# farhiongit/aho-corasick-1975

Hardware: AMD Instinct MI355X
Metric: input GB/s scanned, 1k-keyword dictionary, bit-exact match set (higher is better)
Workload: dtype u8; 1 GPU; BASELINE configs[1]: 1000 ASCII keywords, 1024 MiB synthetic text per GPU (1073741824 symbols of 1 B), 1 keyword planted per 4096 symbols; states=6492, lmax=12, matches_per_gpu=555000, matches_total=555000, parallelism=text sharded x1, 0-symbol halo (the largest any rank used), tables replicated

## Files before the change

aho-corasick-1975_amd/csrc/acm_gpu.hip:

```cpp
#include <hip/hip_runtime.h>
#include <hipcub/hipcub.hpp>

#include <algorithm>
#include <cmath>
#include <cstdint>
#include <cstdio>
#include <cstdlib>
#include <cstring>
#include <mutex>
#include <unordered_map>
#include <vector>

#include "acm_internal.h"

#define HIP_TRY(expr)                                                                              \
  do {                                                                                             \
    hipError_t _e = (expr);                                                                        \
    if (_e != hipSuccess) {                                                                        \
      fprintf (stderr, "acm_gpu: %s failed: %s (%s:%d)\n", #expr, hipGetErrorString (_e), __FILE__, \
               __LINE__);                                                                          \
      return ACM_GPU_E_HIP;                                                                        \
    }                                                                                              \
  } while (0)

// ... 29 lines not shown
enum class PlanKind : uint32_t { Dense = 1, Csr = 2, Sparse = 3, Starts = 4, Gram = 5 };

struct ItemBuffer {
  void *items = nullptr;
  uint32_t *fill = nullptr;
  uint32_t regions = 0, region_items = 0;
};

struct ScanScratch {
  unsigned long long *d_total = nullptr;
  unsigned int *d_pool_ctr = nullptr;
  uint32_t launch_seq = 0;
  void *d_remap = nullptr;
  size_t remap_bytes = 0;
  void *d_holes = nullptr, *d_spill = nullptr;
  uint32_t spill_chunk = 0;
  uint32_t direct_regions = 0;
};

struct ACMPlan {
  int device = 0;
  PlanKind kind = PlanKind::Csr;
  ACMFlatInfo finfo{};
  ACMPlanInfo info{};
  void *blob = nullptr;
  size_t blob_bytes = 0;
  int cu_count = 0;
  uint64_t segment = SEGMENT;
  CsrTables csr{};
  const uint4 *d_oinfo = nullptr;
  const uint32_t *d_kw4 = nullptr;
  const uint16_t *d_cont_dh = nullptr;
  const uint4 *d_chain = nullptr;
  SparseK SK{};
  StartsK TK{};
  StartsMirror *mir = nullptr;
  GramK GK{};
  bool hashed = false, gram2 = false, short_pass = false, short_ids_lds = false, inline_shorts = false;
  uint32_t short_lds_bytes = 0, short_lds_count_bytes = 0;
  uint32_t short_blocks_per_cu = 1;
  uint32_t gram_lds_bytes = 0;
  uint32_t class_sym_bytes = 0;
  bool sparse_lut_lds = false, starts_lut_lds = false;
  uint32_t sparse_lds_bytes = 0, starts_lds_bytes = 0;
  DenseK K{};
  const void *d_dense = nullptr;
  const void *d_lds_image = nullptr;
  const uint32_t *d_wrows = nullptr;
  const uint32_t *d_dstart = nullptr;
  uint32_t lds_image_bytes = 0;
  uint32_t entry_bytes = 0, streams = ACM_DENSE_S, chunk = 64;
  uint16_t *d_classlut = nullptr;
  uint4 *d_intern = nullptr;
  uint32_t intern_mask = 0;
  uint32_t text_sym_bytes = 0;
  bool cls32 = false;
  std::unordered_map<uint32_t, uint32_t> cls32_known;
  std::vector<uint32_t> cls32_reps;
  CMP_TYPE cmp32 = nullptr;
  void *cmp32_arg = nullptr;
  unsigned long long *d_cls32 = nullptr;
  uint32_t cls32_slots = 0, cls32_uploaded = 0;
  uint32_t *d_unknown = nullptr;
  static constexpr uint32_t CLS32_CAP_MIN = 1u << 16, CLS32_CAP_MAX = 1u << 22, CLS32_KNOWN_MAX = 1u << 25;
  uint32_t cls32_cap = CLS32_CAP_MIN;

// ... 462 lines not shown
  memcpy (B.at<uint32_t> (T.o_sym), fv.edge_sym, (size_t)fi.n_edges * 4);
  memcpy (B.at<uint32_t> (T.o_next), fv.edge_next, (size_t)fi.n_edges * 4);
  memcpy (B.at<uint32_t> (T.o_fail), fv.fail, (size_t)n * 4);
  memcpy (B.at<uint32_t> (T.o_cnbo), fv.nb_outputs, (size_t)n * 4);
  uint32_t *oi = B.at<uint32_t> (T.o_oinfo);
  for (uint32_t s = 0; s < n; s++) {
    const uint32_t nb = fv.nb_outputs[s];
    const uint32_t t0 = fv.term_kw[s] != NONE ? s : fv.out_link[s];
    oi[4 * s + 0] = nb;
    oi[4 * s + 1] = nb ? fv.out_link[t0] : 0;
    oi[4 * s + 2] = nb ? fv.depth[t0] : 0;
    oi[4 * s + 3] = nb ? fv.term_kw[t0] + B.kw_base : 0;
  }
  memcpy (B.at<uint32_t> (T.o_dstart), fv.depth_start, ((size_t)fi.lmax + 2) * 4);
}

void
bind_common (ACMPlan *p, const PlanBuild &B, const CommonTables &T, unsigned char *b) {
  auto u32p = [&] (size_t off) { return reinterpret_cast<const uint32_t *> (b + off); };
  p->csr.row_ptr = u32p (T.o_row);
  p->csr.edge_sym = u32p (T.o_sym);
  p->csr.edge_next = u32p (T.o_next);
  p->csr.fail = u32p (T.o_fail);
  p->csr.nb_outputs = u32p (T.o_cnbo);
  p->csr.lmax = B.fi.lmax;
  p->d_oinfo = reinterpret_cast<const uint4 *> (b + T.o_oinfo);
  p->d_dstart = u32p (T.o_dstart);
}

struct DenseTables {
  bool on = false, cont = false;
  uint32_t entry_bytes = 0, rowbytes = 0, queue_bytes = 0, HD = 0, rows_lds = 0, image_bytes = 0;
  std::vector<uint16_t> hotfail;
  size_t o_dense = 0, o_contdh = 0, o_wrows = 0, o_chain = 0, o_image = 0;
};

void
fill_chain_records (const ACMFlatView &fv, uint32_t n, const DenseTables &D, uint32_t *ch) {
  for (uint32_t s0 = D.HD; s0 < n; s0++) {
    uint32_t *r = ch + 4 * (size_t)(s0 - D.HD);
    const uint32_t dh = fv.depth[D.hotfail[s0]];
    if (fv.fail[s0] >= D.HD || dh >= 4000)
      continue;
    uint64_t syms = 0;
    uint32_t len = 0, st = s0;
    bool ok = true;
    while (fv.row_ptr[st + 1] > fv.row_ptr[st]) {
      if (fv.row_ptr[st + 1] - fv.row_ptr[st] != 1 || len == 8 || (st != s0 && fv.term_kw[st] != NONE)) {
        ok = false;
        break;
      }
      syms |= (uint64_t)(fv.edge_sym[fv.row_ptr[st]] & 0xFFu) << (8 * len);
      st = fv.edge_next[fv.row_ptr[st]];
      len++;
    }
    if (!ok)
      continue;
    r[0] = (len ? len : 15u) | (dh << 4);
    r[1] = st;
    r[2] = (uint32_t)syms;
    r[3] = (uint32_t)(syms >> 32);
  }
}

int
build_dense (PlanBuild &B, DenseTables &D) {
  const ACMFlatInfo &fi = B.fi;
  const ACMFlatView &fv = B.fv;
  const uint32_t n = fi.n_states;
  D.entry_bytes = n <= 32768 ? 2 : 4;
  D.on = fi.sym_bytes == 1 && fi.n_edges > 0 && (uint64_t)n * fi.width < (1ull << 31) &&
         (uint64_t)n * fi.width * D.entry_bytes <= (8ull << 30) && fi.lmax >= 1 && fi.lmax - 1 <= 16u * 255;
  D.cont = D.on && D.entry_bytes == 2;
  D.rowbytes = fi.width * D.entry_bytes;
  D.queue_bytes = DENSE_LDS_QUEUE ? (DENSE_THREADS / WAVE) * QCAP * 8 : 0;
  if (D.on) {
    const uint32_t budget = B.lds_cap - D.queue_bytes - 512;
    if (D.cont) {
      const uint64_t fixed = (uint64_t)n * 2;
      D.HD = fixed >= budget ? 1 : (uint32_t)((budget - fixed) / (D.rowbytes - 2));
    } else
      D.HD = budget / D.rowbytes;
    if (D.HD > n)
      D.HD = n;
    if (D.HD < 1)
      D.HD = 1;
  }
  if (D.cont) {
    D.hotfail.resize (n);
    for (uint32_t s = 0; s < n; s++)
      D.hotfail[s] = (uint16_t)(s < D.HD ? s : D.hotfail[fv.fail[s]]);
  }
  D.o_dense = B.reserve ((D.on ? (size_t)n * D.rowbytes : 0) + 16);
  D.o_contdh = B.reserve (D.cont ? (size_t)n * 2 : 0);
  D.o_wrows = B.reserve (D.cont ? (size_t)n * fi.width * 4 : 0);
  D.o_chain = B.reserve (D.cont ? (size_t)(n - D.HD) * 16 + 16 : 0);
  D.rows_lds = D.on ? ((D.HD * D.rowbytes + 15) & ~15u) : 0;
  D.image_bytes = D.on ? ((D.rows_lds + (D.cont ? (n - D.HD) * 2 : 0) + 15) & ~15u) : 0;
  D.o_image = B.reserve (D.image_bytes + 16);
  if (!D.on)
    return ACM_GPU_OK;
  int rc = acm_flat_dense_rows (B.flat, n, D.entry_bytes, B.at<unsigned char> (D.o_dense));
  if (rc)
    return rc;
  memcpy (B.at<unsigned char> (D.o_image), B.at<unsigned char> (D.o_dense), (size_t)D.HD * D.rowbytes);
  if (D.cont) {
    const uint16_t *r16 = B.at<uint16_t> (D.o_dense);
    uint32_t *wr = B.at<uint32_t> (D.o_wrows);
    for (size_t i = 0; i < (size_t)n * fi.width; i++)
      wr[i] = r16[i] | (fv.depth[r16[i] & 0x7FFFu] << 16);
    uint16_t *cdh = B.at<uint16_t> (D.o_contdh);
    for (uint32_t s = 0; s < n; s++)
      cdh[s] = (uint16_t)fv.depth[D.hotfail[s]];
    memcpy (B.at<unsigned char> (D.o_image + D.rows_lds), D.hotfail.data () + D.HD, (size_t)(n - D.HD) * 2);
    fill_chain_records (fv, n, D, B.at<uint32_t> (D.o_chain));
  }
  return ACM_GPU_OK;
}

void
bind_dense (ACMPlan *p, const PlanBuild &B, const DenseTables &D, unsigned char *b) {
  const ACMFlatInfo &fi = B.fi;
  p->entry_bytes = D.entry_bytes;
  if (!D.on)
    return;
  p->kind = PlanKind::Dense;
  p->d_dense = b + D.o_dense;
  p->d_lds_image = b + D.o_image;
  p->d_cont_dh = D.cont ? reinterpret_cast<const uint16_t *> (b + D.o_contdh) : nullptr;
  p->d_chain = D.cont ? reinterpret_cast<const uint4 *> (b + D.o_chain) : nullptr;
  p->d_wrows = D.cont ? reinterpret_cast<const uint32_t *> (b + D.o_wrows) : nullptr;
  p->lds_image_bytes = D.image_bytes;
  DenseK &K = p->K;
  K.W = fi.width;
  K.rowbytes = D.rowbytes;
  K.lo = fi.alpha_lo;
  K.span = fi.alpha_span;
  K.HD = D.HD;
  K.aux_off = D.rows_lds;
  K.queue_off = D.image_bytes;
  K.wub = fi.lmax > 1 ? (fi.lmax - 1 + 15) / 16 : 0;
  K.lmax = fi.lmax;
  K.stream_stride = WAVE * p->chunk;
}

struct GramTables {
  bool on = false;
  bool hashed = false;
// ... 325 lines not shown
  I.grid_blocks = (uint32_t)p->cu_count;
  I.block_threads = SPARSE_THREADS;
  switch (p->kind) {
  case PlanKind::Dense:
    I.lds_bytes = D.image_bytes + D.queue_bytes + 16 ;
    I.block_threads = DENSE_THREADS;
    break;
  case PlanKind::Csr:
    I.lds_bytes = QCAP * 8;
    I.block_threads = WAVE;
    I.grid_blocks = (uint32_t)p->cu_count * 16;
    break;
  case PlanKind::Sparse:
  case PlanKind::Starts:
    I.lds_bytes = p->kind == PlanKind::Starts ? p->starts_lds_bytes : p->sparse_lds_bytes;
    I.streams = p->kind == PlanKind::Starts ? 1 : SPARSE_S;
    I.chunk_bytes = 128;
    break;
  case PlanKind::Gram:
    I.lds_bytes = p->gram_lds_bytes;
    I.streams = 1;
    I.chunk_bytes = 16;
    break;
  }
}

int
build_tables (PlanBuild &B, ACMPlan *p) {
  CommonTables T;
  DenseTables D;
  SparseTables S;
  GramTables G;
  build_common (B, T);
  int rc = build_dense (B, D);
  if (rc)
    return rc;
  build_sparse (B, D, S);
  rc = build_gram (B, D, G);
  if (rc)
    return rc;
  const size_t bytes = B.host.size ();
  p->blob_bytes = bytes;
  if (hipMalloc (&p->blob, bytes) != hipSuccess)
    return ACM_GPU_E_NOMEM;
  if (hipMemcpy (p->blob, B.host.data (), bytes, hipMemcpyHostToDevice) != hipSuccess)
    return ACM_GPU_E_HIP;
  const size_t ctl_bytes = 16 + 2 * POOL_CLASSES * POOL_CTR_STRIDE * sizeof (unsigned int);
  if (hipMalloc (reinterpret_cast<void **> (&p->scratch.d_total), ctl_bytes) != hipSuccess || hipMemset (p->scratch.d_total, 0, ctl_bytes) != hipSuccess)
    return ACM_GPU_E_NOMEM;
  p->scratch.d_pool_ctr = reinterpret_cast<unsigned int *> (p->scratch.d_total + 2);
  unsigned char *b = static_cast<unsigned char *> (p->blob);
  bind_common (p, B, T, b);
  bind_dense (p, B, D, b);
  bind_gram (p, B, G, b);
  bind_sparse (p, B, S, T.o_oinfo, b);
  fill_plan_info (p, D);
  return ACM_GPU_OK;
}

int
set_lds_attributes (const ACMPlan *p) {
  for (int co = 0; co < 2; co++) {
    switch (p->kind) {
    case PlanKind::Dense:
      HIP_TRY (hipFuncSetAttribute (dense_kernel (p, co != 0), hipFuncAttributeMaxDynamicSharedMemorySize,
                                    (int)p->info.lds_bytes));
      break;
    case PlanKind::Starts:
      HIP_TRY (hipFuncSetAttribute (starts_kernel (p, co != 0), hipFuncAttributeMaxDynamicSharedMemorySize,
                                    (int)p->starts_lds_bytes));
      [[fallthrough]];
    case PlanKind::Sparse:
      HIP_TRY (hipFuncSetAttribute (sparse_kernel (p, co != 0), hipFuncAttributeMaxDynamicSharedMemorySize,
                                    (int)p->sparse_lds_bytes));
      break;
    case PlanKind::Gram:
      HIP_TRY (hipFuncSetAttribute (gram_kernel (p, co != 0, false), hipFuncAttributeMaxDynamicSharedMemorySize,
                                    (int)p->gram_lds_bytes));
      if (p->short_pass)
        HIP_TRY (hipFuncSetAttribute (short_kernel (p, co != 0), hipFuncAttributeMaxDynamicSharedMemorySize,
                                      (int)(co ? p->short_lds_count_bytes : p->short_lds_bytes)));
      break;
    case PlanKind::Csr: break;
// ... 139 lines not shown
    return rc;
  rc = acm_gpu_plan_create_flat (flat, device, out);
  acm_flat_release (flat);
  if (!rc) {
    (*out)->class_sym_bytes = sym_bytes;
    if ((*out)->cls32)
      acm_internal_comparator (machine, &(*out)->cmp32, &(*out)->cmp32_arg);
  }
  return rc;
}

extern "C" void
acm_gpu_plan_destroy (ACMPlan *plan) {
  if (!plan)
    return;
  (void)hipSetDevice (plan->device);
  if (plan->delta || !plan->retired.empty ())
    (void)hipDeviceSynchronize ();
  for (auto &r : plan->retired) {
    if (r.done)
      (void)hipEventDestroy (r.done);
    acm_gpu_plan_destroy (r.plan);
  }
  plan->retired.clear ();
  if (plan->delta)
    acm_gpu_plan_destroy (plan->delta);
  plan->delta = nullptr;
  for (auto &ev : plan->events) {
    (void)hipEventDestroy (ev.start);
    (void)hipEventDestroy (ev.scan_done);
    (void)hipEventDestroy (ev.all_done);
  }
  void *const owned[] = { plan->blob, plan->own_items.items, plan->own_items.fill, plan->scratch.d_holes, plan->scratch.d_spill, plan->scratch.d_total,
                          plan->scratch.d_remap, plan->d_intern, plan->d_cls32, plan->d_unknown, plan->d_classlut };
  for (void *d : owned)
    if (d)
      (void)hipFree (d);
  if (plan->mir) {
    if (plan->mir->own)
      for (int t = 0; t < 5; t++)
        if (t != PT_LUT && plan->mir->dev[t])
          (void)hipFree (plan->mir->dev[t]);
    if (plan->mir->d_patches)
      (void)hipFree (plan->mir->d_patches);
    delete plan->mir;
  }
  delete plan;
}

extern "C" void
acm_gpu_plan_info (const ACMPlan *plan, ACMPlanInfo *info) {
  *info = plan->info;
  info->delta_keywords = plan->delta ? plan->delta->finfo.n_keywords : 0;
  info->merges = plan->merges;
  const bool gram = plan->kind == PlanKind::Gram;
  info->records_direct = ((gram && !plan->hashed) || plan->kind == PlanKind::Csr) ? 1u : 0u;
  info->variant = gram ? (plan->gram2 ? 2u : 0u) | (plan->short_pass ? 4u : 0u) | (plan->short_pass && !plan->short_ids_lds ? 8u : 0u) : 0u;
}

extern "C" int
acm_gpu_plan_status (ACMPlan *plan) {
  if (!plan)
    return ACM_GPU_E_ARG;
  HIP_TRY (hipSetDevice (plan->device));
  HIP_TRY (hipDeviceSynchronize ());
  if (!plan->scratch.d_total)
    return ACM_GPU_OK;
// ... 324 lines not shown
    buf->fill = nullptr;
    if (hipMalloc (&buf->items, (size_t)regions * per * 8) != hipSuccess)
      return ACM_GPU_E_NOMEM;
    if (hipMalloc (reinterpret_cast<void **> (&buf->fill), (size_t)regions * 4) != hipSuccess)
      return ACM_GPU_E_NOMEM;
    HIP_TRY (hipMemset (buf->fill, 0, (size_t)regions * 4));
    HIP_TRY (hipDeviceSynchronize ());
    buf->regions = regions;
    buf->region_items = (uint32_t)per;
  }
  return ACM_GPU_OK;
}

int
ensure_direct_buffers (ACMPlan *p, uint32_t rec_chunk) {
  const uint32_t regions = (uint32_t)p->cu_count * (SPARSE_THREADS / WAVE);
  if (p->scratch.d_holes && p->scratch.d_spill && p->scratch.direct_regions >= regions && p->scratch.spill_chunk >= rec_chunk)
    return ACM_GPU_OK;
  if (p->scratch.d_holes || p->scratch.d_spill)
    HIP_TRY (hipDeviceSynchronize ());
  if (p->scratch.d_holes)
    HIP_TRY (hipFree (p->scratch.d_holes));
  if (p->scratch.d_spill)
    HIP_TRY (hipFree (p->scratch.d_spill));
  p->scratch.d_holes = p->scratch.d_spill = nullptr;
  if (hipMalloc (&p->scratch.d_holes, (size_t)regions * 2 * sizeof (RecHole)) != hipSuccess ||
      hipMalloc (&p->scratch.d_spill, (size_t)regions * rec_chunk * 16) != hipSuccess)
    return ACM_GPU_E_NOMEM;
  p->scratch.direct_regions = regions;
  p->scratch.spill_chunk = rec_chunk;
  return ACM_GPU_OK;
}

template <bool CONT, bool COUNT_ONLY>
void
launch_expand_cfg (ACMPlan *p, const EmitCtx &E, uint32_t regions_used, const ExpandTail &tail, hipStream_t st) {
  const dim3 g ((regions_used + 15) / 16);
  const ItemBuffer &I = p->items ();
  hipLaunchKernelGGL ((expand_items_once_kernel<CONT, COUNT_ONLY, 1024, 16, 4>), g, dim3 (1024), 0, st, E,
                      static_cast<const uint2 *> (I.items), I.region_items, I.fill, tail);
}

template <bool COUNT_ONLY>
int
launch_dense (ACMPlan *p, const EmitCtx &E, Launch a, hipStream_t st, hipEvent_t stop, uint64_t *d_count, bool last_segment) {
  const uint32_t TILE = WAVE * p->streams * p->chunk;
  a.range_begin = 0;
  a.range_end = (uint32_t)(((uint64_t)a.n + TILE - 1) / TILE);
  uint32_t grid = p->info.grid_blocks;
  const uint32_t wpb = DENSE_THREADS / WAVE;
  const uint32_t blocks_needed = (a.range_end + wpb - 1) / wpb;
  if (blocks_needed < grid)
    grid = blocks_needed;
  static_assert (DENSE_THREADS == SPARSE_THREADS, "set_tile_pool counts blocks of SPARSE_THREADS");
  set_tile_pool (p, a, grid * wpb);
  ItemBuffer &I = p->items ();
  void *args[] = { &p->K, const_cast<EmitCtx *> (&E), &a, &p->d_dense, &p->d_lds_image, &p->lds_image_bytes, &a.text,
                   &I.items, &I.region_items, &I.fill, &p->d_dstart };
  HIP_TRY (hipLaunchKernel (dense_kernel (p, COUNT_ONLY), dim3 (grid), dim3 (DENSE_THREADS), args, p->info.lds_bytes, st));
  if (stop)
    HIP_TRY (hipEventRecord (stop, st));
  ExpandTail tail;
  tail.user_count = reinterpret_cast<unsigned long long *> (d_count);
  tail.ticket = reinterpret_cast<unsigned int *> (p->scratch.d_total + 1);
  tail.last_segment = last_segment ? 1 : 0;
  if (p->entry_bytes == 2)
    launch_expand_cfg<true, COUNT_ONLY> (p, E, grid * wpb, tail, st);
  else
    launch_expand_cfg<false, COUNT_ONLY> (p, E, grid * wpb, tail, st);
  HIP_TRY (hipGetLastError ());
  return ACM_GPU_OK;
}

int
starts_flush (ACMPlan *p, hipStream_t st) {
  StartsMirror &M = *p->mir;
  if (M.full_upload) {
    HIP_TRY (hipDeviceSynchronize ());
    uint32_t *fresh[5] = { nullptr, nullptr, nullptr, nullptr, nullptr };
    size_t want[5];
    for (int t = 0; t < 5; t++) {
      if (t == PT_LUT)
        continue;
      want[t] = M.tab[t].size () * 2 + 4096;
      const bool keep = M.own && M.cap[t] >= M.tab[t].size ();
      if (keep)
        fresh[t] = M.dev[t];
      else if (hipMalloc (reinterpret_cast<void **> (&fresh[t]), want[t] * 4) != hipSuccess ||
               hipMemset (fresh[t], 0, want[t] * 4) != hipSuccess) {
        for (int u = 0; u <= t; u++)
          if (fresh[u] && fresh[u] != M.dev[u])
            (void)hipFree (fresh[u]);
        return ACM_GPU_E_NOMEM;
      }
    }
    for (int t = 0; t < 5; t++) {
      if (t == PT_LUT) {
// ... 623 lines not shown
    HIP_TRY (hipEventRecord (s->copied[cur], s->copy));
    const uint64_t ctx = s->prev_valid < s->halo ? s->prev_valid : s->halo;
    HIP_TRY (hipStreamWaitEvent (s->compute, s->copied[cur], 0));
    if (ctx) {
      const unsigned char *tail = s->slot[prev] + (s->halo + s->last_piece - ctx) * s->sb;
      HIP_TRY (hipMemcpyAsync (piece_at - ctx * s->sb, tail, (size_t)ctx * s->sb, hipMemcpyDeviceToDevice, s->compute));
    }
    HIP_TRY (hipEventRecord (s->tail_read[prev], s->compute));
    int rc = scan_plan<false> (p, piece_at - ctx * s->sb, ctx + n, ctx, s->position - ctx, s->d_records, s->capacity, nullptr,
                               s->compute, true);
    if (rc)
      return rc;
    HIP_TRY (hipEventRecord (s->scanned[cur], s->compute));
    s->prev_valid = ctx + n;
    s->last_piece = n;
    s->position += n;
    s->pieces++;
    src += (size_t)n * s->sb;
    n_symbols -= n;
  }
  return ACM_GPU_OK;
}

extern "C" int
acm_gpu_stream_finish (ACMStream *s, ACMRecord *records, uint64_t capacity, uint64_t *n_found) {
  if (!s || !n_found)
    return ACM_GPU_E_ARG;
  ACMPlan *p = s->plan;
  HIP_TRY (hipSetDevice (p->device));
  HIP_TRY (hipStreamSynchronize (s->copy));
  HIP_TRY (hipStreamSynchronize (s->compute));
  unsigned long long total = 0;
  HIP_TRY (hipMemcpy (&total, p->scratch.d_total, 8, hipMemcpyDeviceToHost));
  *n_found = total;
  if (total > s->capacity || total > capacity)
    return ACM_GPU_E_OVERFLOW;
  if (total > 1) {
    const size_t tb = acm_gpu_order_tmp_bytes (p, total, s->position);
    void *tmp = nullptr;
    if (hipMalloc (&tmp, tb) != hipSuccess)
      return ACM_GPU_E_NOMEM;
    int rc = acm_gpu_order_records_device (p, s->d_records, total, 0, s->position, tmp, tb, s->compute);
    if (!rc && hipStreamSynchronize (s->compute) != hipSuccess)
      rc = ACM_GPU_E_HIP;
    (void)hipFree (tmp);
    if (rc)
      return rc;
  }
  if (total && records)
    HIP_TRY (hipMemcpy (records, s->d_records, total * sizeof (ACMRecord), hipMemcpyDeviceToHost));
  return acm_gpu_plan_status (p);
}

extern "C" void
acm_gpu_stream_close (ACMStream *s) {
  if (!s)
    return;
  (void)hipSetDevice (s->plan->device);
  if (s->copy)
    (void)hipStreamSynchronize (s->copy);
  if (s->compute)
    (void)hipStreamSynchronize (s->compute);
  (void)hipMemset (s->plan->scratch.d_total, 0, 8);
  (void)hipDeviceSynchronize ();
  for (int i = 0; i < 2; i++) {
    if (s->slot[i]) (void)hipFree (s->slot[i]);
// ... 1026 lines not shown
```

aho-corasick-1975_amd/csrc/dev_emit.h:

```cpp

__device__ __forceinline__ uint32_t
lane_id () {
  return __builtin_amdgcn_mbcnt_hi (~0u, __builtin_amdgcn_mbcnt_lo (~0u, 0u));
}

__device__ __forceinline__ uint32_t
rank_below (uint64_t m) {
  return __builtin_amdgcn_mbcnt_hi ((uint32_t)(m >> 32), __builtin_amdgcn_mbcnt_lo ((uint32_t)m, 0u));
}

__device__ __forceinline__ uint32_t
lshl_or (uint32_t a, uint32_t s, uint32_t b) {
  uint32_t r;
  asm ("v_lshl_or_b32 %0, %1, %2, %3" : "=v"(r) : "v"(a), "v"(s), "v"(b));
  return r;
}

__device__ __forceinline__ uint32_t
uniform (uint32_t v) {
  return __builtin_amdgcn_readfirstlane (v);
}

__device__ __forceinline__ uint32_t
wave_incl_scan (uint32_t v) {
// ... 66 lines not shown
      }
      return r;
    }
  }
  const uint32_t dh = walk ? 0u : E.cont_dh[st];
  uint32_t s2 = st;
  uint32_t byte = pos + 1 < E.n ? E.text[pos + 1] : 0;
  for (uint32_t j = 1; pos + j < E.n; j++) {
    const uint32_t p = pos + j;
    const uint32_t ent = E.wrows[s2 * E.W + min (byte - E.lo, E.span)];
    byte = p + 1 < E.n ? E.text[p + 1] : 0;
    s2 = ent & IT_STATE;
    const uint32_t past = p + 1 > ce ? p + 1 - ce : 0;
    const uint32_t bound = j + dh > past ? j + dh : past;
    if ((ent >> 16) <= bound)
      break;
    if ((ent & 0x8000u) && p >= E.emit_from) {
      const uint4 oi = E.oinfo[s2];
      const uint32_t c = put_outputs<WRITE> (E, oi, p, bound, o + r.cnt);
      if (c) {
        if (!r.events) {
          r.ev_pos = p;
          r.ev_oi = oi;
          r.ev_bound = bound;
        }
        r.events++;
        r.cnt += c;
      }
    }
  }
  return r;
}

template <bool CONT>
__device__ __forceinline__ uint32_t
item_count (const EmitCtx &E, bool valid, uint2 it, uint32_t &own_cnt, uint4 &own_oi, ContResult &r) {
  const uint32_t st = CONT ? (it.y & IT_STATE) : it.y;
  if (valid && st >= E.n_states) {
    if (E.error)
      *E.error = 1;
    valid = false;
  }
  const bool own = valid && (!CONT || (it.y & IT_OUT));
  own_cnt = 0;
  own_oi = make_uint4 (0, 0, 0, 0);
  if (own) {
    own_oi = E.oinfo[st];
    if (CONT && (it.y & IT_RUN))
      own_cnt = put_outputs<false> (E, own_oi, it.x, (it.y >> IT_K_SHIFT) & 0xFFFu, 0);
    else
      own_cnt = own_oi.x;
  }
  r = ContResult{ 0, 0, 0, 0, make_uint4 (0, 0, 0, 0) };
  if (CONT && valid && (it.y & IT_CONT))
    r = walk_continuation<false> (E, it, 0);
  return own_cnt + r.cnt;
}

template <bool CONT>
__device__ __forceinline__ void
item_write (const EmitCtx &E, uint2 it, uint32_t own_cnt, uint4 own_oi, const ContResult &r, uint64_t o) {
  if (own_cnt)
    (void)put_outputs<true> (E, own_oi, it.x, (CONT && (it.y & IT_RUN)) ? ((it.y >> IT_K_SHIFT) & 0xFFFu) : 0u, o);
  if (r.events == 1)
    (void)put_outputs<true> (E, r.ev_oi, r.ev_pos, r.ev_bound, o + own_cnt);
  else if (r.events > 1)
// ... 50 lines not shown
  if (m) {
    if (hit)
      queue[qn + rank_below (m)] = make_uint2 (pos, word);
    qn = uniform (qn + (uint32_t)__popcll (m));
    if (qn > QCAP - WAVE) {
      queue_drain<CONT, COUNT_ONLY, PARK_ONLY> (E, queue, qn, sp, lane);
      qn = 0;
    }
  }
}

__device__ __forceinline__ void
region_push (Spill *sp, bool hit, uint32_t pos, uint32_t word) {
  const uint64_t m = __ballot (hit);
  if (m) {
    if (hit)
      sp->region[sp->fill + rank_below (m)] = make_uint2 (pos, word);
    sp->fill = uniform (sp->fill + (uint32_t)__popcll (m));
  }
}

template <bool CONT, bool COUNT_ONLY, int S>
__device__ __forceinline__ void
region_make_room (const EmitCtx &E, Spill *sp) {
  if (sp->capacity - sp->fill < 16u * S * WAVE + QCAP) {
    __builtin_amdgcn_fence (__ATOMIC_RELEASE, "workgroup");
    asm volatile ("s_waitcnt vmcnt(0)" ::: "memory");
    flush_queue<CONT, COUNT_ONLY> (E, sp->region, sp->fill);
    asm volatile ("s_waitcnt vmcnt(0)" ::: "memory");
    sp->fill = 0;
  }
}

struct ExpandTail {
  unsigned long long *user_count;
  unsigned int *ticket;
  int last_segment;
};

template <bool CONT, bool COUNT_ONLY, int THREADS, int REGIONS>
__global__ __launch_bounds__ (THREADS) void
expand_items_kernel (EmitCtx E, const uint2 *items, uint32_t region_items, uint32_t *fill, ExpandTail tail) {
  __shared__ uint32_t s_off[REGIONS + 1];
  __shared__ uint32_t s_wave[THREADS / WAVE];
  __shared__ unsigned long long s_base;
  const uint32_t tid = threadIdx.x, lane = tid & (WAVE - 1), wid = tid / WAVE;
  if (tid < REGIONS) {
    s_off[tid + 1] = fill[blockIdx.x * REGIONS + tid];
    fill[blockIdx.x * REGIONS + tid] = 0;
  }
  __syncthreads ();
  if (tid == 0) {
    uint32_t acc = 0;
    for (int r = 0; r < REGIONS; r++) {
      const uint32_t v = s_off[r + 1];
      s_off[r] = acc;
      acc += v;
    }
    s_off[REGIONS] = acc;
  }
  __syncthreads ();
  const uint32_t total = s_off[REGIONS];
  for (uint32_t base = 0; base < total; base += THREADS) {
    const uint32_t i = base + tid;
    const bool valid = i < total;
    uint2 it = make_uint2 (0, 0);
    if (valid) {
      uint32_t r = 0;
#pragma unroll
      for (int k = 1; k < REGIONS; k++)
        r += s_off[k] <= i ? 1u : 0u;
      it = items[(size_t)(blockIdx.x * REGIONS + r) * region_items + (i - s_off[r])];
    }
    uint32_t own_cnt;
    uint4 own_oi;
    ContResult res;
    const uint32_t cnt = item_count<CONT> (E, valid, it, own_cnt, own_oi, res);
    const uint32_t incl = wave_incl_scan (cnt);
    if (lane == WAVE - 1)
      s_wave[wid] = incl;
    __syncthreads ();
    if (tid == 0) {
      uint32_t acc = 0;
      for (int k = 0; k < THREADS / WAVE; k++) {
        const uint32_t v = s_wave[k];
        s_wave[k] = acc;
        acc += v;
      }
      s_base = acc ? atomicAdd (E.count, (unsigned long long)acc) : 0ull;
    }
    __syncthreads ();
    if (!COUNT_ONLY && cnt)
      item_write<CONT> (E, it, own_cnt, own_oi, res, s_base + s_wave[wid] + (incl - cnt));
    __syncthreads ();
  }
  if (tid == 0) {
    if (atomicAdd (tail.ticket, 1u) == gridDim.x - 1) {
      *tail.ticket = 0;
      if (tail.last_segment) {
        *tail.user_count = atomicAdd (E.count, 0ull);
        *E.count = 0;
      }
    }
  }
}

template <bool CONT, bool COUNT_ONLY, int THREADS, int REGIONS, int ROUNDS>
__global__ __launch_bounds__ (THREADS) void
expand_items_once_kernel (EmitCtx E, const uint2 *items, uint32_t region_items, uint32_t *fill, ExpandTail tail) {
  constexpr int WAVES = THREADS / WAVE;
  __shared__ uint32_t s_off[REGIONS + 1];
  __shared__ uint32_t s_wave[ROUNDS][WAVES];
  __shared__ unsigned long long s_base;
  const uint32_t tid = threadIdx.x, lane = tid & (WAVE - 1), wid = tid / WAVE;
  if (tid < REGIONS) {
    s_off[tid + 1] = fill[blockIdx.x * REGIONS + tid];
    fill[blockIdx.x * REGIONS + tid] = 0;
  }
  __syncthreads ();
  if (tid == 0) {
    uint32_t acc = 0;
    for (int r = 0; r < REGIONS; r++) {
      const uint32_t v = s_off[r + 1];
      s_off[r] = acc;
      acc += v;
    }
    s_off[REGIONS] = acc;
  }
  __syncthreads ();
  const uint32_t total = s_off[REGIONS];
  for (uint32_t base = 0; base < total; base += THREADS * ROUNDS) {
    uint2 it[ROUNDS];
    uint32_t cnt[ROUNDS], own_cnt[ROUNDS], incl[ROUNDS];
    uint4 own_oi[ROUNDS];
    ContResult res[ROUNDS];
#pragma unroll
    for (int k = 0; k < ROUNDS; k++) {
      const uint32_t i = base + k * THREADS + tid;
      const bool valid = i < total;
      it[k] = make_uint2 (0, 0);
      if (valid) {
        uint32_t r = 0;
#pragma unroll
        for (int j = 1; j < REGIONS; j++)
          r += s_off[j] <= i ? 1u : 0u;
        it[k] = items[(size_t)(blockIdx.x * REGIONS + r) * region_items + (i - s_off[r])];
      }
    }
#pragma unroll
    for (int k = 0; k < ROUNDS; k++) {
      const bool valid = base + k * THREADS + tid < total;
      cnt[k] = item_count<CONT> (E, valid, it[k], own_cnt[k], own_oi[k], res[k]);
      incl[k] = wave_incl_scan (cnt[k]);
      if (lane == WAVE - 1)
        s_wave[k][wid] = incl[k];
    }
    __syncthreads ();
    if (tid == 0) {
      uint32_t acc = 0;
      for (int k = 0; k < ROUNDS; k++)
        for (int w = 0; w < WAVES; w++) {
          const uint32_t v = s_wave[k][w];
          s_wave[k][w] = acc;
          acc += v;
        }
      s_base = acc ? atomicAdd (E.count, (unsigned long long)acc) : 0ull;
    }
    __syncthreads ();
    if (!COUNT_ONLY) {
#pragma unroll
      for (int k = 0; k < ROUNDS; k++)
        if (cnt[k])
          item_write<CONT> (E, it[k], own_cnt[k], own_oi[k], res[k], s_base + s_wave[k][wid] + (incl[k] - cnt[k]));
    }
    __syncthreads ();
  }
  if (tid == 0) {
    if (atomicAdd (tail.ticket, 1u) == gridDim.x - 1) {
      *tail.ticket = 0;
      if (tail.last_segment) {
        *tail.user_count = atomicAdd (E.count, 0ull);
        *E.count = 0;
      }
    }
  }
}
```

aho-corasick-1975_amd/csrc/dev_misc.h:

```cpp

__global__ __launch_bounds__ (1024) void
classmap_kernel (const uint4 *__restrict__ in, uint4 *__restrict__ out, uint64_t n_blocks16, const uint16_t *__restrict__ lut) {
  extern __shared__ __attribute__ ((aligned (16))) unsigned char smem[];
  {
    uint4 *dst = reinterpret_cast<uint4 *> (smem);
    const uint4 *src = reinterpret_cast<const uint4 *> (lut);
    for (uint32_t i = threadIdx.x; i < 65536 * 2 / 16; i += blockDim.x)
      dst[i] = src[i];
  }
  __syncthreads ();
  const uint16_t *l = reinterpret_cast<const uint16_t *> (smem);
  auto map2 = [&] (uint32_t w) -> uint32_t { return (uint32_t)l[w & 0xFFFFu] | ((uint32_t)l[w >> 16] << 16); };
  for (uint64_t i = (uint64_t)blockIdx.x * blockDim.x + threadIdx.x; i < n_blocks16; i += (uint64_t)gridDim.x * blockDim.x) {
    const uint4 v = in[i];
    out[i] = make_uint4 (map2 (v.x), map2 (v.y), map2 (v.z), map2 (v.w));
  }
}

template <typename SYM>
__global__ void
classmap_tail_kernel (const SYM *__restrict__ in, SYM *__restrict__ out, uint64_t begin, uint64_t n, const uint16_t *__restrict__ lut) {
  for (uint64_t i = begin + (uint64_t)blockIdx.x * blockDim.x + threadIdx.x; i < n; i += (uint64_t)gridDim.x * blockDim.x)
    out[i] = (SYM)lut[in[i]];
}
// ... 105 lines not shown
}

__device__ __forceinline__ uint64_t
splitmix64 (uint64_t x) {
  x += 0x9E3779B97F4A7C15ull;
  x = (x ^ (x >> 30)) * 0xBF58476D1CE4E5B9ull;
  x = (x ^ (x >> 27)) * 0x94D049BB133111EBull;
  return x ^ (x >> 31);
}

template <typename SYM>
__global__ void
synth_text_kernel (SYM *text, uint64_t n, uint64_t gbegin, uint32_t vocab, const SYM *kw, const uint32_t *kw_off, uint32_t n_kw) {
  constexpr uint64_t P = 4096;
  const uint64_t stride = (uint64_t)gridDim.x * blockDim.x;
  for (uint64_t li = (uint64_t)blockIdx.x * blockDim.x + threadIdx.x; li < n; li += stride) {
    const uint64_t i = gbegin + li;
    const uint64_t p = i & ~(P - 1);
    uint64_t v = sizeof (SYM) == 1 ? (uint64_t)'a' + splitmix64 (i + 42) % 26 : splitmix64 (i + 42) % vocab;
    if (n_kw) {
      const uint64_t off = p + splitmix64 (p) % (P - 16);
      const uint32_t k = (uint32_t)(splitmix64 (p + 99) % n_kw);
      const uint32_t len = kw_off[k + 1] - kw_off[k];
      if (i >= off && i < off + len)
        v = kw[kw_off[k] + (i - off)];
    }
    text[li] = (SYM)v;
  }
}

__global__ void
finish_count_kernel (unsigned long long *total, unsigned long long *user_count) {
  if (threadIdx.x == 0 && blockIdx.x == 0) {
    *user_count = *total;
    *total = 0;
  }
}
```

Baseline: 3777 GB/s.

## Restructure expand kernel: wave-per-region, fused ticket counter, precomputed chain output info

The expand kernel now gives each wave its own region and reads the first slots unconditionally, so the block-wide serial prefix over region fills and the per-item region search both go away. The grid-completion ticket is packed into the high bits of the global match counter, so each block needs one atomic instead of two; readers mask off the ticket bits. Chain-record output info is precomputed on the host into a new device table, so a matched chain emits directly without walking the continuation. Items beyond the first few rounds per region fall to a separate per-wave path. Costs are more registers, an extra table, and a tighter coupling between region capacity and the kernel template.

```diff
diff --git a/aho-corasick-1975_amd/csrc/acm_gpu.hip b/aho-corasick-1975_amd/csrc/acm_gpu.hip
--- a/aho-corasick-1975_amd/csrc/acm_gpu.hip
+++ b/aho-corasick-1975_amd/csrc/acm_gpu.hip
@@ -85,6 +85,7 @@
   const uint32_t *d_kw4 = nullptr;
   const uint16_t *d_cont_dh = nullptr;
   const uint4 *d_chain = nullptr;
+  uint4 *d_chain_oi = nullptr;
   SparseK SK{};
   StartsK TK{};
   StartsMirror *mir = nullptr;
@@ -613,11 +614,12 @@
   bool on = false, cont = false;
   uint32_t entry_bytes = 0, rowbytes = 0, queue_bytes = 0, HD = 0, rows_lds = 0, image_bytes = 0;
   std::vector<uint16_t> hotfail;
+  std::vector<uint32_t> chain_oi;
   size_t o_dense = 0, o_contdh = 0, o_wrows = 0, o_chain = 0, o_image = 0;
 };
 
 void
-fill_chain_records (const ACMFlatView &fv, uint32_t n, const DenseTables &D, uint32_t *ch) {
+fill_chain_records (const ACMFlatView &fv, uint32_t n, const DenseTables &D, const uint32_t *oinfo, uint32_t *ch, uint32_t *chain_oi) {
   for (uint32_t s0 = D.HD; s0 < n; s0++) {
     uint32_t *r = ch + 4 * (size_t)(s0 - D.HD);
     const uint32_t dh = fv.depth[D.hotfail[s0]];
@@ -641,11 +643,12 @@
     r[1] = st;
     r[2] = (uint32_t)syms;
     r[3] = (uint32_t)(syms >> 32);
+    memcpy (chain_oi + 4 * (size_t)(s0 - D.HD), oinfo + 4 * (size_t)st, 16);
   }
 }
 
 int
-build_dense (PlanBuild &B, DenseTables &D) {
+build_dense (PlanBuild &B, DenseTables &D, size_t oinfo_off) {
   const ACMFlatInfo &fi = B.fi;
   const ACMFlatView &fv = B.fv;
   const uint32_t n = fi.n_states;
@@ -694,7 +697,8 @@
     for (uint32_t s = 0; s < n; s++)
       cdh[s] = (uint16_t)fv.depth[D.hotfail[s]];
     memcpy (B.at<unsigned char> (D.o_image + D.rows_lds), D.hotfail.data () + D.HD, (size_t)(n - D.HD) * 2);
-    fill_chain_records (fv, n, D, B.at<uint32_t> (D.o_chain));
+    D.chain_oi.assign (4 * (size_t)(n - D.HD) + 4, 0);
+    fill_chain_records (fv, n, D, B.at<uint32_t> (oinfo_off), B.at<uint32_t> (D.o_chain), D.chain_oi.data ());
   }
   return ACM_GPU_OK;
 }
@@ -1086,7 +1090,7 @@
   SparseTables S;
   GramTables G;
   build_common (B, T);
-  int rc = build_dense (B, D);
+  int rc = build_dense (B, D, T.o_oinfo);
   if (rc)
     return rc;
   build_sparse (B, D, S);
@@ -1103,6 +1107,13 @@
   if (hipMalloc (reinterpret_cast<void **> (&p->scratch.d_total), ctl_bytes) != hipSuccess || hipMemset (p->scratch.d_total, 0, ctl_bytes) != hipSuccess)
     return ACM_GPU_E_NOMEM;
   p->scratch.d_pool_ctr = reinterpret_cast<unsigned int *> (p->scratch.d_total + 2);
+  if (!D.chain_oi.empty ()) {
+    const size_t oi_bytes = D.chain_oi.size () * sizeof (uint32_t);
+    if (hipMalloc (reinterpret_cast<void **> (&p->d_chain_oi), oi_bytes) != hipSuccess)
+      return ACM_GPU_E_NOMEM;
+    if (hipMemcpy (p->d_chain_oi, D.chain_oi.data (), oi_bytes, hipMemcpyHostToDevice) != hipSuccess)
+      return ACM_GPU_E_HIP;
+  }
   unsigned char *b = static_cast<unsigned char *> (p->blob);
   bind_common (p, B, T, b);
   bind_dense (p, B, D, b);
@@ -1308,7 +1319,7 @@
     (void)hipEventDestroy (ev.all_done);
   }
   void *const owned[] = { plan->blob, plan->own_items.items, plan->own_items.fill, plan->scratch.d_holes, plan->scratch.d_spill, plan->scratch.d_total,
-                          plan->scratch.d_remap, plan->d_intern, plan->d_cls32, plan->d_unknown, plan->d_classlut };
+                          plan->d_chain_oi, plan->scratch.d_remap, plan->d_intern, plan->d_cls32, plan->d_unknown, plan->d_classlut };
   for (void *d : owned)
     if (d)
       (void)hipFree (d);
@@ -1699,13 +1710,18 @@
   return ACM_GPU_OK;
 }
 
+#ifndef ACM_EXPAND_WAVES
+#define ACM_EXPAND_WAVES 16
+#endif
 template <bool CONT, bool COUNT_ONLY>
 void
 launch_expand_cfg (ACMPlan *p, const EmitCtx &E, uint32_t regions_used, const ExpandTail &tail, hipStream_t st) {
-  const dim3 g ((regions_used + 15) / 16);
+  constexpr int WAVES = ACM_EXPAND_WAVES;
+  const dim3 g ((regions_used + WAVES - 1) / WAVES);
   const ItemBuffer &I = p->items ();
-  hipLaunchKernelGGL ((expand_items_once_kernel<CONT, COUNT_ONLY, 1024, 16, 4>), g, dim3 (1024), 0, st, E,
-                      static_cast<const uint2 *> (I.items), I.region_items, I.fill, tail);
+  hipLaunchKernelGGL ((expand_items_once_kernel<CONT, COUNT_ONLY, WAVES * WAVE, WAVES, 4>), g, dim3 (WAVES * WAVE), 0, st, E,
+                      static_cast<const uint2 *> (I.items), I.region_items, I.fill, regions_used,
+                      static_cast<const uint4 *> (p->d_chain_oi), tail);
 }
 
 template <bool COUNT_ONLY>
@@ -1729,7 +1745,6 @@
     HIP_TRY (hipEventRecord (stop, st));
   ExpandTail tail;
   tail.user_count = reinterpret_cast<unsigned long long *> (d_count);
-  tail.ticket = reinterpret_cast<unsigned int *> (p->scratch.d_total + 1);
   tail.last_segment = last_segment ? 1 : 0;
   if (p->entry_bytes == 2)
     launch_expand_cfg<true, COUNT_ONLY> (p, E, grid * wpb, tail, st);
@@ -2419,6 +2434,7 @@
   HIP_TRY (hipStreamSynchronize (s->compute));
   unsigned long long total = 0;
   HIP_TRY (hipMemcpy (&total, p->scratch.d_total, 8, hipMemcpyDeviceToHost));
+  total &= EXPAND_TOTAL_MASK;
   *n_found = total;
   if (total > s->capacity || total > capacity)
     return ACM_GPU_E_OVERFLOW;
diff --git a/aho-corasick-1975_amd/csrc/dev_emit.h b/aho-corasick-1975_amd/csrc/dev_emit.h
--- a/aho-corasick-1975_amd/csrc/dev_emit.h
+++ b/aho-corasick-1975_amd/csrc/dev_emit.h
@@ -122,6 +122,37 @@
   return r;
 }
 
+__device__ __forceinline__ bool
+item_has_chain (const EmitCtx &E, uint2 it) {
+  return E.chain && !(it.y & IT_WALK) && (it.y & IT_STATE) >= E.chain_base && it.x + 9 <= E.n;
+}
+
+__device__ __forceinline__ bool
+chain_hit (const EmitCtx &E, uint32_t pos, uint32_t ce, uint4 c, uint64_t have, uint32_t &p, uint32_t &bound) {
+  const uint32_t len = c.x & 15u;
+  const uint64_t want = ((uint64_t)c.w << 32) | c.z;
+  p = pos + len;
+  if (len == 15u || ((want ^ have) << (64u - 8u * len)) != 0 || p < E.emit_from)
+    return false;
+  const uint32_t past = p + 1 > ce ? p + 1 - ce : 0, jd = len + (c.x >> 4);
+  bound = jd > past ? jd : past;
+  return true;
+}
+
+__device__ __forceinline__ ContResult
+chain_result (const EmitCtx &E, uint32_t p, uint32_t bound, uint4 leaf_oi) {
+  ContResult r = { 0, 0, 0, 0, make_uint4 (0, 0, 0, 0) };
+  const uint32_t cnt = put_outputs<false> (E, leaf_oi, p, bound, 0);
+  if (cnt) {
+    r.ev_pos = p;
+    r.ev_oi = leaf_oi;
+    r.ev_bound = bound;
+    r.events = 1;
+    r.cnt = cnt;
+  }
+  return r;
+}
+
 template <bool CONT>
 __device__ __forceinline__ uint32_t
 item_count (const EmitCtx &E, bool valid, uint2 it, uint32_t &own_cnt, uint4 &own_oi, ContResult &r) {
@@ -238,156 +269,151 @@
   }
 }
 
+constexpr int EXPAND_TICKET_SHIFT = 48;
+constexpr unsigned long long EXPAND_TOTAL_MASK = (1ull << EXPAND_TICKET_SHIFT) - 1;
+
+template <bool CONT, bool COUNT_ONLY>
+__device__ __forceinline__ void
+expand_rest (EmitCtx E, const uint2 *queue, uint32_t n_items) {
+  const uint32_t lane = lane_id ();
+  for (uint32_t base = 0; base < n_items; base += WAVE) {
+    const uint32_t i = base + lane;
+    const bool valid = i < n_items;
+    const uint2 it = valid ? queue[i] : make_uint2 (0, 0);
+    uint32_t own_cnt;
+    uint4 own_oi;
+    ContResult r;
+    const uint32_t cnt = item_count<CONT> (E, valid, it, own_cnt, own_oi, r);
+    const uint32_t incl = wave_incl_scan (cnt);
+    const uint32_t total = __shfl (incl, WAVE - 1, WAVE);
+    unsigned long long gbase = 0;
+    if (lane == 0 && total)
+      gbase = atomicAdd (E.count, (unsigned long long)total) & EXPAND_TOTAL_MASK;
+    gbase = ((unsigned long long)__shfl ((uint32_t)(gbase >> 32), 0, WAVE) << 32) | __shfl ((uint32_t)gbase, 0, WAVE);
+    if (!COUNT_ONLY && cnt)
+      item_write<CONT> (E, it, own_cnt, own_oi, r, gbase + (incl - cnt));
+  }
+  __threadfence ();
+}
+
 struct ExpandTail {
   unsigned long long *user_count;
-  unsigned int *ticket;
   int last_segment;
 };
 
-template <bool CONT, bool COUNT_ONLY, int THREADS, int REGIONS>
-__global__ __launch_bounds__ (THREADS) void
-expand_items_kernel (EmitCtx E, const uint2 *items, uint32_t region_items, uint32_t *fill, ExpandTail tail) {
-  __shared__ uint32_t s_off[REGIONS + 1];
-  __shared__ uint32_t s_wave[THREADS / WAVE];
-  __shared__ unsigned long long s_base;
-  const uint32_t tid = threadIdx.x, lane = tid & (WAVE - 1), wid = tid / WAVE;
-  if (tid < REGIONS) {
-    s_off[tid + 1] = fill[blockIdx.x * REGIONS + tid];
-    fill[blockIdx.x * REGIONS + tid] = 0;
-  }
-  __syncthreads ();
-  if (tid == 0) {
-    uint32_t acc = 0;
-    for (int r = 0; r < REGIONS; r++) {
-      const uint32_t v = s_off[r + 1];
-      s_off[r] = acc;
-      acc += v;
-    }
-    s_off[REGIONS] = acc;
-  }
-  __syncthreads ();
-  const uint32_t total = s_off[REGIONS];
-  for (uint32_t base = 0; base < total; base += THREADS) {
-    const uint32_t i = base + tid;
-    const bool valid = i < total;
-    uint2 it = make_uint2 (0, 0);
-    if (valid) {
-      uint32_t r = 0;
-#pragma unroll
-      for (int k = 1; k < REGIONS; k++)
-        r += s_off[k] <= i ? 1u : 0u;
-      it = items[(size_t)(blockIdx.x * REGIONS + r) * region_items + (i - s_off[r])];
-    }
-    uint32_t own_cnt;
-    uint4 own_oi;
-    ContResult res;
-    const uint32_t cnt = item_count<CONT> (E, valid, it, own_cnt, own_oi, res);
-    const uint32_t incl = wave_incl_scan (cnt);
-    if (lane == WAVE - 1)
-      s_wave[wid] = incl;
-    __syncthreads ();
-    if (tid == 0) {
-      uint32_t acc = 0;
-      for (int k = 0; k < THREADS / WAVE; k++) {
-        const uint32_t v = s_wave[k];
-        s_wave[k] = acc;
-        acc += v;
-      }
-      s_base = acc ? atomicAdd (E.count, (unsigned long long)acc) : 0ull;
-    }
-    __syncthreads ();
-    if (!COUNT_ONLY && cnt)
-      item_write<CONT> (E, it, own_cnt, own_oi, res, s_base + s_wave[wid] + (incl - cnt));
-    __syncthreads ();
-  }
-  if (tid == 0) {
-    if (atomicAdd (tail.ticket, 1u) == gridDim.x - 1) {
-      *tail.ticket = 0;
-      if (tail.last_segment) {
-        *tail.user_count = atomicAdd (E.count, 0ull);
-        *E.count = 0;
-      }
-    }
-  }
-}
-
 template <bool CONT, bool COUNT_ONLY, int THREADS, int REGIONS, int ROUNDS>
 __global__ __launch_bounds__ (THREADS) void
-expand_items_once_kernel (EmitCtx E, const uint2 *items, uint32_t region_items, uint32_t *fill, ExpandTail tail) {
+expand_items_once_kernel (EmitCtx E, const uint2 *items, uint32_t region_items, uint32_t *fill, uint32_t n_regions,
+                          const uint4 *chain_oi, ExpandTail tail) {
   constexpr int WAVES = THREADS / WAVE;
-  __shared__ uint32_t s_off[REGIONS + 1];
-  __shared__ uint32_t s_wave[ROUNDS][WAVES];
-  __shared__ unsigned long long s_base;
-  const uint32_t tid = threadIdx.x, lane = tid & (WAVE - 1), wid = tid / WAVE;
-  if (tid < REGIONS) {
-    s_off[tid + 1] = fill[blockIdx.x * REGIONS + tid];
-    fill[blockIdx.x * REGIONS + tid] = 0;
-  }
+  static_assert (WAVES == REGIONS, "wave w of a block expands region w");
+  static_assert (ROUNDS * WAVES <= WAVE, "every wave scans the wave totals with one LDS read per lane");
+  static_assert (ROUNDS * WAVE <= (int)DENSE_MIN_REGION_ITEMS, "the first slots are read whatever the fill");
+  __shared__ uint32_t s_wave[ROUNDS * WAVES];
+  __shared__ unsigned long long s_old;
+  const uint32_t lane = lane_id (), wid = uniform (threadIdx.x / WAVE);
+  DIAG (unsigned long long d_t[8]; int d_n = 0;)
+#define ACM_STAMP() DIAG (asm volatile ("s_waitcnt vmcnt(0) lgkmcnt(0)" ::: "memory"); d_t[d_n++] = wall_clock64 ();)
+  ACM_STAMP ()
+  const uint32_t region = blockIdx.x * REGIONS + wid;
+  const bool have_region = region < n_regions;
+  const uint2 *src = items + (size_t)(have_region ? region : 0u) * region_items;
+  const uint32_t fill_raw = __hip_atomic_load (&fill[have_region ? region : 0u], __ATOMIC_RELAXED, __HIP_MEMORY_SCOPE_AGENT);
+  uint2 it[ROUNDS];
+#pragma unroll
+  for (int k = 0; k < ROUNDS; k++)
+    it[k] = src[k * WAVE + lane];
+  if (have_region && lane == 0)
+    fill[region] = 0;
+  const uint32_t nfill = have_region ? uniform (fill_raw) : 0u;
+  ACM_STAMP ()
+  if (nfill > ROUNDS * WAVE)
+    expand_rest<CONT, COUNT_ONLY> (E, src + ROUNDS * WAVE, nfill - ROUNDS * WAVE);
+
+  uint4 own_oi[ROUNDS], cc[ROUNDS], coi[ROUNDS];
+  uint64_t have[ROUNDS];
+  uint32_t vmask = 0;
+#pragma unroll
+  for (int k = 0; k < ROUNDS; k++) {
+    bool valid = k * WAVE + lane < nfill;
+    if (valid && (CONT ? (it[k].y & IT_STATE) : it[k].y) >= E.n_states) {
+      if (E.error)
+        *E.error = 1;
+      valid = false;
+    }
+    if (!valid)
+      it[k] = make_uint2 (0, 0);
+    vmask |= (valid ? 1u : 0u) << k;
+    const uint32_t st = CONT ? (it[k].y & IT_STATE) : it[k].y;
+    const bool own = CONT ? (it[k].y & IT_OUT) != 0 : valid;
+    own_oi[k] = E.oinfo[own ? st : 0u];
+    if (CONT) {
+      const bool ch = (it[k].y & IT_CONT) && item_has_chain (E, it[k]);
+      const uint32_t ci = ch ? st - E.chain_base : 0u;
+      cc[k] = E.chain[ci];
+      coi[k] = chain_oi[ci];
+      __builtin_memcpy (&have[k], E.text + (ch ? it[k].x + 1 : 0u), 8);
+    }
+  }
+  ACM_STAMP ()
+
+  uint32_t cnt[ROUNDS], own_cnt[ROUNDS], incl[ROUNDS];
+  ContResult res[ROUNDS];
+#pragma unroll
+  for (int k = 0; k < ROUNDS; k++) {
+    if (!(CONT ? (it[k].y & IT_OUT) != 0 : (vmask >> k & 1u) != 0))
+      own_cnt[k] = 0;
+    else if (CONT && (it[k].y & IT_RUN))
+      own_cnt[k] = put_outputs<false> (E, own_oi[k], it[k].x, (it[k].y >> IT_K_SHIFT) & 0xFFFu, 0);
+    else
+      own_cnt[k] = own_oi[k].x;
+    res[k] = ContResult{ 0, 0, 0, 0, make_uint4 (0, 0, 0, 0) };
+    if (CONT && (it[k].y & IT_CONT)) {
+      if (item_has_chain (E, it[k]) && (cc[k].x & 15u)) {
+        uint32_t p, bound;
+        if (chain_hit (E, it[k].x, item_chunk_end (E, it[k]), cc[k], have[k], p, bound))
+          res[k] = chain_result (E, p, bound, coi[k]);
+      } else
+        res[k] = walk_continuation<false> (E, it[k], 0);
+    }
+    cnt[k] = own_cnt[k] + res[k].cnt;
+    incl[k] = wave_incl_scan (cnt[k]);
+    if (lane == WAVE - 1)
+      s_wave[k * WAVES + wid] = incl[k];
+  }
+  ACM_STAMP ()
   __syncthreads ();
-  if (tid == 0) {
-    uint32_t acc = 0;
-    for (int r = 0; r < REGIONS; r++) {
-      const uint32_t v = s_off[r + 1];
-      s_off[r] = acc;
-      acc += v;
-    }
-    s_off[REGIONS] = acc;
-  }
+  const uint32_t wt = lane < ROUNDS * WAVES ? s_wave[lane] : 0u;
+  const uint32_t before = wave_incl_scan (wt) - wt;
+  const uint32_t acc = __shfl (before + wt, WAVE - 1, WAVE);
+  ACM_STAMP ()
+  if (threadIdx.x == 0)
+    s_old = atomicAdd (E.count, (unsigned long long)acc + (1ull << EXPAND_TICKET_SHIFT));
   __syncthreads ();
-  const uint32_t total = s_off[REGIONS];
-  for (uint32_t base = 0; base < total; base += THREADS * ROUNDS) {
-    uint2 it[ROUNDS];
-    uint32_t cnt[ROUNDS], own_cnt[ROUNDS], incl[ROUNDS];
-    uint4 own_oi[ROUNDS];
-    ContResult res[ROUNDS];
+  const unsigned long long old = s_old;
+  ACM_STAMP ()
+  if (!COUNT_ONLY) {
 #pragma unroll
     for (int k = 0; k < ROUNDS; k++) {
-      const uint32_t i = base + k * THREADS + tid;
-      const bool valid = i < total;
-      it[k] = make_uint2 (0, 0);
-      if (valid) {
-        uint32_t r = 0;
-#pragma unroll
-        for (int j = 1; j < REGIONS; j++)
-          r += s_off[j] <= i ? 1u : 0u;
-        it[k] = items[(size_t)(blockIdx.x * REGIONS + r) * region_items + (i - s_off[r])];
-      }
-    }
-#pragma unroll
-    for (int k = 0; k < ROUNDS; k++) {
-      const bool valid = base + k * THREADS + tid < total;
-      cnt[k] = item_count<CONT> (E, valid, it[k], own_cnt[k], own_oi[k], res[k]);
-      incl[k] = wave_incl_scan (cnt[k]);
-      if (lane == WAVE - 1)
-        s_wave[k][wid] = incl[k];
-    }
-    __syncthreads ();
-    if (tid == 0) {
-      uint32_t acc = 0;
-      for (int k = 0; k < ROUNDS; k++)
-        for (int w = 0; w < WAVES; w++) {
-          const uint32_t v = s_wave[k][w];
-          s_wave[k][w] = acc;
-          acc += v;
-        }
-      s_base = acc ? atomicAdd (E.count, (unsigned long long)acc) : 0ull;
-    }
-    __syncthreads ();
-    if (!COUNT_ONLY) {
-#pragma unroll
-      for (int k = 0; k < ROUNDS; k++)
-        if (cnt[k])
-          item_write<CONT> (E, it[k], own_cnt[k], own_oi[k], res[k], s_base + s_wave[k][wid] + (incl[k] - cnt[k]));
-    }
-    __syncthreads ();
-  }
-  if (tid == 0) {
-    if (atomicAdd (tail.ticket, 1u) == gridDim.x - 1) {
-      *tail.ticket = 0;
-      if (tail.last_segment) {
-        *tail.user_count = atomicAdd (E.count, 0ull);
-        *E.count = 0;
-      }
-    }
-  }
-}
+      const uint32_t wave_off = __shfl (before, k * WAVES + wid, WAVE);
+      if (cnt[k])
+        item_write<CONT> (E, it[k], own_cnt[k], own_oi[k], res[k], (old & EXPAND_TOTAL_MASK) + wave_off + (incl[k] - cnt[k]));
+    }
+  }
+  if (threadIdx.x == 0 && (old >> EXPAND_TICKET_SHIFT) == gridDim.x - 1) {
+    if (tail.last_segment) {
+      *tail.user_count = (old & EXPAND_TOTAL_MASK) + acc;
+      *E.count = 0;
+    } else
+      (void)atomicAdd (E.count, 0ull - ((unsigned long long)gridDim.x << EXPAND_TICKET_SHIFT));
+  }
+  ACM_STAMP ()
+  DIAG (if (threadIdx.x == 0 && (blockIdx.x == 0 || blockIdx.x == gridDim.x / 2)) {
+    unsigned long long *o = g_acm_diag[4096 + (blockIdx.x ? 1 : 0)];
+    for (int i = 0; i < 6; i++)
+      o[i] = d_t[i + 1] - d_t[i];
+    o[6] = d_t[6] - d_t[0];
+    o[7] = nfill;
+  })
+#undef ACM_STAMP
+}
diff --git a/aho-corasick-1975_amd/csrc/dev_misc.h b/aho-corasick-1975_amd/csrc/dev_misc.h
--- a/aho-corasick-1975_amd/csrc/dev_misc.h
+++ b/aho-corasick-1975_amd/csrc/dev_misc.h
@@ -161,7 +161,7 @@
 __global__ void
 finish_count_kernel (unsigned long long *total, unsigned long long *user_count) {
   if (threadIdx.x == 0 && blockIdx.x == 0) {
-    *user_count = *total;
+    *user_count = *total & EXPAND_TOTAL_MASK;
     *total = 0;
   }
 }
```

Result: no change. 3788 GB/s, median of 6 (+0.3%).
